# speechcatcher-asr/speechcatcher

Hardware: AMD Instinct MI355X
Metric: concurrent real-time streams (audio-seconds/s), de_xl dims, 640 ms (10240-sample) chunk steps, beam 10 CTC+attention (higher is better)
Workload: dtype f32

## Files before the change

speechcatcher_amd/csrc/gemm.hip:

```cpp
#define SC_STAMP_ON (p.dbg_stamp)
#include "common.h"
#include <mutex>
#include <unordered_map>
#include <vector>

typedef float f32x16 __attribute__((ext_vector_type(16)));
typedef _Float16 h16x4 __attribute__((ext_vector_type(4)));
typedef _Float16 h16x8 __attribute__((ext_vector_type(8)));

__device__ __forceinline__ void ffn_split4(const float4 &x, h16x4 &hi, h16x4 &lo) {
  hi = h16x4{(_Float16)x.x, (_Float16)x.y, (_Float16)x.z, (_Float16)x.w};
  lo = h16x4{(_Float16)((x.x - (float)hi[0]) * 2048.f), (_Float16)((x.y - (float)hi[1]) * 2048.f),
             (_Float16)((x.z - (float)hi[2]) * 2048.f), (_Float16)((x.w - (float)hi[3]) * 2048.f)};
}

struct GemmArgs {
  const float *A;
  const int *a_rows;
  int lda;
  const float *W;
  const float *bias;
  float *C;
  const int *c_rows;
  int ldc;
// ... 745 lines not shown
               "not a tiled problem");
  if (M == 0) return SC_OK;
  hipStream_t st = (hipStream_t)stream;
  resolve_workspace(stream);
  if (sc_hook("SC_GEMM_NAIVE") || sc_hook("SC_SKINNY_MAX_M") || sc_hook("SC_KV_PER_LAYER")) return SC_ERR_ARG;
  ProfScope prof = sc_prof_begin(st);
  GemmArgs g{A, a_rows, lda, W, bias, C, c_rows, ldc, M, N, K, flags, 0, nullptr, K, ncb, cb_stride};
  int ksplit = 0, variant = 0;
  float *ws_keep = g_ws;
  g_ws = nullptr;
  gemm_dispatch(g, false, &ksplit, &variant, st);
  g_ws = ws_keep;
  sc_prof_end(prof, variant, 2.0 * M * N * K, 4.0 * ((double)M * K + (double)N * K + (double)M * N));
  SC_CHECK_LAUNCH();
  return SC_OK;
}

extern "C" int sc_gemm_ln(const float *A, const int32_t *a_rows, int lda, const float *W,
                          const float *bias, float *C, const int32_t *c_rows, int ldc, int M, int N,
                          int K, int flags, int conv_f1, const float *ln_g, const float *ln_b,
                          float ln_eps, float *ln_out, int ld_ln, void *stream) {
  SC_CHECK_ARG(A && W && C && ln_g && ln_b && ln_out, "null pointer");
  SC_CHECK_ARG(M >= 0 && N > 0 && K > 0 && lda > 0 && ldc >= N && ld_ln >= N, "bad dimensions");
  if (M == 0) return SC_OK;
  GemmArgs g{A, a_rows, lda, W, bias, C, c_rows, ldc, M, N, K, flags, conv_f1, nullptr, K};
  hipStream_t st = (hipStream_t)stream;
  resolve_workspace(stream);
  const bool fusable = N <= 1024 && N % 4 == 0 && ld_ln % 4 == 0;
  int ksplit = 0, variant = 0;
  gemm_dispatch(g, fusable, &ksplit, &variant, st);
  if (ksplit > 0 && fusable) {
    gemm_splitk_reduce_ln_kernel<<<cdiv(M, 4), 256, 0, st>>>(g, ksplit, ln_g, ln_b, ln_eps, ln_out, ld_ln);
    SC_CHECK_LAUNCH();
    return SC_OK;
  }
  if (ksplit > 0) {
    const long n4 = (long)M * (N / 4);
    gemm_splitk_reduce_kernel<<<dim3((unsigned)((n4 + 255) / 256)), 256, 0, st>>>(g, ksplit);
  }
  SC_CHECK_LAUNCH();
  return sc_layernorm(C, c_rows, ldc, ln_out, (flags & SC_GEMM_LN_AT_CROWS) ? c_rows : nullptr, ld_ln, M, N, ln_g,
                      ln_b, ln_eps, stream);
}

typedef float f32x4 __attribute__((ext_vector_type(4)));

__device__ __forceinline__ f32x4 ffn_mfma8(f32x4 acc, const float4 &a0, const float4 &a1, const float4 &b0,
                                           const float4 &b1) {
  acc = __builtin_amdgcn_mfma_f32_16x16x4f32(a0.x, b0.x, acc, 0, 0, 0);
  acc = __builtin_amdgcn_mfma_f32_16x16x4f32(a0.y, b0.y, acc, 0, 0, 0);
  acc = __builtin_amdgcn_mfma_f32_16x16x4f32(a0.z, b0.z, acc, 0, 0, 0);
  acc = __builtin_amdgcn_mfma_f32_16x16x4f32(a0.w, b0.w, acc, 0, 0, 0);
  acc = __builtin_amdgcn_mfma_f32_16x16x4f32(a1.x, b1.x, acc, 0, 0, 0);
  acc = __builtin_amdgcn_mfma_f32_16x16x4f32(a1.y, b1.y, acc, 0, 0, 0);
  acc = __builtin_amdgcn_mfma_f32_16x16x4f32(a1.z, b1.z, acc, 0, 0, 0);
  acc = __builtin_amdgcn_mfma_f32_16x16x4f32(a1.w, b1.w, acc, 0, 0, 0);
  return acc;
}

struct FfnArgs {
  const float *XN;
  const int *rows;
  const float *W1p, *b1, *W2p;
  float *part;
  int M, F, cpw;
  const float *PH;
  int nph;
  const float *pbias, *Xin;
  float *Xout;
  const float *g, *b;
  float eps;
  int part_rows;
  int w_form;
  int act_half;
  int dbg_stamp;
  int pgrp;
};

__device__ __forceinline__ f32x4 ffn_mma_h(f32x4 acc, const h16x8 &a, const h16x4 &b0, const h16x4 &b1) {
  acc = __builtin_amdgcn_mfma_f32_16x16x16f16(h16x4{a[0], a[1], a[2], a[3]}, b0, acc, 0, 0, 0);
  acc = __builtin_amdgcn_mfma_f32_16x16x16f16(h16x4{a[4], a[5], a[6], a[7]}, b1, acc, 0, 0, 0);
  return acc;
}
__host__ __device__ static inline size_t ffn_lds_bytes(int D, int RT, bool pro, int wf) {
  const bool wh = wf == 1;
  if (!wh) return (size_t)(RT * (D + 4) + RT * (128 + 4) + (pro ? RT : 0)) * sizeof(float);
  return (size_t)RT * (D + 4) * 4 + (size_t)RT * (D + 8) * 2 + (size_t)RT * (128 + 8) * 2 + (pro ? RT * 4 : 0);
}

template <int D, int RTT, bool PRO = false, int WF = 0>
__global__ __launch_bounds__(512) void ffn_fused_kernel(FfnArgs p) {
  constexpr bool WH = WF == 1, WS = WF == 2;
  constexpr int RT = 16 * RTT, FC = 128;
  constexpr int KI1 = D / 32, KI2 = FC / 32, NT2 = D / 128;
  constexpr int LDX = D + 4, LDH = FC + 4;
  constexpr int LDXH = D + 8, LDHH = FC + 8;
  constexpr int LDXS = 2 * D + 8, LDHS = 2 * FC + 8;
  extern __shared__ __attribute__((aligned(16))) float ffn_smem[];
  float *Xs = ffn_smem;
  float *Hs = ffn_smem + RT * LDX;
  _Float16 *XsH = reinterpret_cast<_Float16 *>(ffn_smem + RT * LDX);
  _Float16 *HsH = XsH + RT * LDXH;
  int *rowid = WH ? reinterpret_cast<int *>(HsH + RT * LDHH)
                  : reinterpret_cast<int *>(ffn_smem + RT * LDX + RT * LDH);
  _Float16 *XsS = reinterpret_cast<_Float16 *>(ffn_smem);
  _Float16 *HsS = reinterpret_cast<_Float16 *>(ffn_smem + RT * LDX);
  typedef typename std::conditional<WS, h16x8, typename std::conditional<WH, h16x4, float4>::type>::type BF;
  auto split_at = [](int c) { return (c >> 3) * 16 + (c & 7); };
  const int lane = threadIdx.x & 63, wave = threadIdx.x >> 6;
  const int r = lane & 15, kk = lane >> 4;
  const int grp = blockIdx.x, m0 = blockIdx.y * RT;
  const int KF = p.F / 32;

  constexpr int NV = RT * D / 4;
  constexpr int NQ = NV / 512;
  static_assert(NV % 512 == 0, "tile must be a multiple of the workgroup");
  SC_STAMP(PRO ? 2 : 3, 0);
  BF bf[KI1][2];
  auto load_b1 = [&](int chunk) {
    const BF *wp = reinterpret_cast<const BF *>(p.W1p) + ((long)(chunk * 8 + wave) * KI1) * 128 + lane;
#pragma unroll
    for (int ki = 0; ki < KI1; ++ki) {
      bf[ki][0] = wp[ki * 128];
      bf[ki][1] = wp[ki * 128 + 64];
    }
  };
  BF b2f[KI2][NT2][2];
  auto load_b2 = [&](int chunk) {
#pragma unroll
    for (int t = 0; t < NT2; ++t) {
      const BF *wp = reinterpret_cast<const BF *>(p.W2p) +
                         ((long)(wave * NT2 + t) * KF + chunk * KI2) * 128 + lane;
#pragma unroll
      for (int k = 0; k < KI2; ++k) {
        b2f[k][t][0] = wp[k * 128];
        b2f[k][t][1] = wp[k * 128 + 64];
      }
    }
  };
  if (PRO) {
    constexpr int C4 = D / 4, Q4 = D / 64;
    const int sub = threadIdx.x & 15;
    float4 gam[Q4], bet[Q4];
#pragma unroll
    for (int q = 0; q < Q4; ++q) {
      gam[q] = *reinterpret_cast<const float4 *>(p.g + 4 * (sub + 16 * q));
      bet[q] = *reinterpret_cast<const float4 *>(p.b + 4 * (sub + 16 * q));
    }
    long rowv[NQ];
#pragma unroll
    for (int q = 0; q < NQ; ++q) {
      const int m = min(m0 + (threadIdx.x + q * 512) / C4, p.M - 1);
      rowv[q] = p.rows ? p.rows[m] : m;
    }
    SC_STAMP_WAIT(2, 1);
#pragma unroll
    for (int q = 0; q < NQ; ++q) {
      const int e = threadIdx.x + q * 512, i = e / C4, c4 = e % C4;
      const long row = rowv[q];
      if (c4 == 0) rowid[i] = (int)row;
      const float4 xi = *reinterpret_cast<const float4 *>(p.Xin + row * D + 4 * c4);
      float4 pb = make_float4(0.f, 0.f, 0.f, 0.f);
      if (p.pbias) pb = *reinterpret_cast<const float4 *>(p.pbias + 4 * c4);
      float4 y = make_float4(0.f, 0.f, 0.f, 0.f);
      auto ldp = [&](long elem) -> float4 {
        if (p.act_half) {
          const h16x4 h = *reinterpret_cast<const h16x4 *>(reinterpret_cast<const _Float16 *>(p.PH) + elem);
          return make_float4((float)h[0], (float)h[1], (float)h[2], (float)h[3]);
        }
        return *reinterpret_cast<const float4 *>(p.PH + elem);
      };
      if (p.pgrp == 1 && p.nph == 2) {
        const float4 p0 = ldp((row * 2) * D + 4 * c4);
        const float4 p1 = ldp((row * 2 + 1) * D + 4 * c4);
        y = sc_add4(p0, p1);
      } else
      for (int z0 = 0; z0 < p.nph; z0 += 8) {
        float4 pv[8];
#pragma unroll
        for (int z = 0; z < 8; ++z) {
          pv[z] = ldp((row * p.nph + min(z0 + z, p.nph - 1)) * D + 4 * c4);
          if (z0 + z >= p.nph) pv[z] = make_float4(0.f, 0.f, 0.f, 0.f);
        }
        if (p.pgrp == 4) {
          const float4 g0 = sc_seq4(pv[0], pv[1], pv[2], pv[3]);
          y = z0 == 0 ? g0 : sc_add4(y, g0);
          if (z0 + 4 < p.nph) y = sc_add4(y, sc_seq4(pv[4], pv[5], pv[6], pv[7]));
        } else {
#pragma unroll
          for (int z = 0; z < 8; ++z)
            if (z0 + z < p.nph) y = (z0 + z == 0) ? pv[0] : sc_add4(y, pv[z]);
        }
      }
      const float4 x = make_float4(xi.x + (y.x + pb.x), xi.y + (y.y + pb.y), xi.z + (y.z + pb.z), xi.w + (y.w + pb.w));
      if (grp == 0 && m0 + i < p.M) *reinterpret_cast<float4 *>(p.Xout + row * D + 4 * c4) = x;
      *reinterpret_cast<float4 *>(Xs + i * LDX + 4 * c4) = x;
    }
    SC_STAMP_WAIT(2, 2);
    load_b1(grp * p.cpw);
    __syncthreads();
    SC_STAMP(2, 3);
    for (int i = threadIdx.x >> 4; i < RT; i += 32) {
      float4 x[Q4];
      float sum = 0.f;
#pragma unroll
      for (int q = 0; q < Q4; ++q) {
        x[q] = *reinterpret_cast<const float4 *>(Xs + i * LDX + 4 * (sub + 16 * q));
        sum += (x[q].x + x[q].y) + (x[q].z + x[q].w);
      }
      const float mean = group_sum<16>(sum) / (float)D;
      float q2 = 0.f;
#pragma unroll
      for (int q = 0; q < Q4; ++q) {
        const float a = x[q].x - mean, b = x[q].y - mean, c = x[q].z - mean, e = x[q].w - mean;
        q2 += (a * a + b * b) + (c * c + e * e);
      }
      const float rstd = 1.0f / sqrtf(group_sum<16>(q2) / (float)D + p.eps);
#pragma unroll
      for (int q = 0; q < Q4; ++q) {
        const float4 o = make_float4((x[q].x - mean) * rstd * gam[q].x + bet[q].x, (x[q].y - mean) * rstd * gam[q].y + bet[q].y,
                                     (x[q].z - mean) * rstd * gam[q].z + bet[q].z, (x[q].w - mean) * rstd * gam[q].w + bet[q].w);
        if (WS) {
          h16x4 hi, lo;
          ffn_split4(o, hi, lo);
          _Float16 *d = XsS + i * LDXS + split_at(4 * (sub + 16 * q));
          *reinterpret_cast<h16x4 *>(d) = hi;
          *reinterpret_cast<h16x4 *>(d + 8) = lo;
        } else if (WH)
          *reinterpret_cast<h16x4 *>(XsH + i * LDXH + 4 * (sub + 16 * q)) =
              h16x4{(_Float16)o.x, (_Float16)o.y, (_Float16)o.z, (_Float16)o.w};
        else
          *reinterpret_cast<float4 *>(Xs + i * LDX + 4 * (sub + 16 * q)) = o;
      }
    }
    SC_STAMP(2, 4);
  } else {
    long rowv[NQ];
#pragma unroll
    for (int q = 0; q < NQ; ++q) {
      const int m = min(m0 + (threadIdx.x + q * 512) / (D / 4), p.M - 1);
      rowv[q] = p.rows ? p.rows[m] : m;
    }
    float4 stage[NQ];
#pragma unroll
    for (int q = 0; q < NQ; ++q)
      stage[q] = *reinterpret_cast<const float4 *>(p.XN + rowv[q] * D + 4 * ((threadIdx.x + q * 512) % (D / 4)));
#pragma unroll
    for (int q = 0; q < NQ; ++q) {
      const int e = threadIdx.x + q * 512;
      if (WS) {
        h16x4 hi, lo;
        ffn_split4(stage[q], hi, lo);
        _Float16 *d = XsS + (e / (D / 4)) * LDXS + split_at(4 * (e % (D / 4)));
        *reinterpret_cast<h16x4 *>(d) = hi;
        *reinterpret_cast<h16x4 *>(d + 8) = lo;
      } else if (WH)
        *reinterpret_cast<h16x4 *>(XsH + (e / (D / 4)) * LDXH + 4 * (e % (D / 4))) =
            h16x4{(_Float16)stage[q].x, (_Float16)stage[q].y, (_Float16)stage[q].z, (_Float16)stage[q].w};
      else
        *reinterpret_cast<float4 *>(Xs + (e / (D / 4)) * LDX + 4 * (e % (D / 4))) = stage[q];
    }
  }
  f32x4 acc2[RTT][NT2];
  f32x4 acc2c[WS ? RTT : 1][WS ? NT2 : 1];
#pragma unroll
  for (int rt = 0; rt < RTT; ++rt)
#pragma unroll
    for (int t = 0; t < NT2; ++t) {
      acc2[rt][t] = f32x4{0.f, 0.f, 0.f, 0.f};
      if (WS) acc2c[rt][t] = f32x4{0.f, 0.f, 0.f, 0.f};
    }

  if (!PRO) load_b1(grp * p.cpw);
  __syncthreads();
  SC_STAMP(PRO ? 2 : 3, PRO ? 5 : 1);
  if (PRO) SC_STAMP_WAIT(2, 6);

  for (int cc = 0; cc < p.cpw; ++cc) {
    const int chunk = grp * p.cpw + cc;
    const float bias = p.b1 ? p.b1[chunk * FC + wave * 16 + r] : 0.f;
    load_b2(chunk);
    f32x4 acc1[RTT];
    f32x4 acc1c[WS ? RTT : 1];
#pragma unroll
    for (int rt = 0; rt < RTT; ++rt) {
      acc1[rt] = f32x4{0.f, 0.f, 0.f, 0.f};
      if (WS) acc1c[rt] = f32x4{0.f, 0.f, 0.f, 0.f};
    }
    if constexpr (WS) {
      constexpr int NS = RTT * KI1;
      const _Float16 *ab = XsS + r * LDXS + 16 * kk;
      h16x8 ah = *reinterpret_cast<const h16x8 *>(ab), al = *reinterpret_cast<const h16x8 *>(ab + 8);
#pragma unroll
      for (int st = 0; st < NS; ++st) {
        const int ki = st / RTT, rt = st % RTT;
        h16x8 nh = ah, nl = al;
        if (st + 1 < NS) {
          const _Float16 *ap = ab + ((st + 1) % RTT) * 16 * LDXS + ((st + 1) / RTT) * 64;
          nh = *reinterpret_cast<const h16x8 *>(ap);
          nl = *reinterpret_cast<const h16x8 *>(ap + 8);
        }
        acc1[rt] = __builtin_amdgcn_mfma_f32_16x16x32_f16(ah, bf[ki][0], acc1[rt], 0, 0, 0);
        acc1c[rt] = __builtin_amdgcn_mfma_f32_16x16x32_f16(ah, bf[ki][1], acc1c[rt], 0, 0, 0);
        acc1c[rt] = __builtin_amdgcn_mfma_f32_16x16x32_f16(al, bf[ki][0], acc1c[rt], 0, 0, 0);
        ah = nh;
        al = nl;
      }
    } else if constexpr (WH) {
      constexpr int NS = RTT * KI1;
      const _Float16 *ab = XsH + r * LDXH + 8 * kk;
      h16x8 a = *reinterpret_cast<const h16x8 *>(ab);
#pragma unroll
      for (int st = 0; st < NS; ++st) {
        const int ki = st / RTT, rt = st % RTT;
        h16x8 n = a;
        if (st + 1 < NS) n = *reinterpret_cast<const h16x8 *>(ab + ((st + 1) % RTT) * 16 * LDXH + ((st + 1) / RTT) * 32);
        acc1[rt] = ffn_mma_h(acc1[rt], a, bf[ki][0], bf[ki][1]);
        a = n;
      }
    } else {
      constexpr int NS = RTT * KI1;
      const float *ab = Xs + r * LDX + 8 * kk;
      float4 a0 = *reinterpret_cast<const float4 *>(ab), a1 = *reinterpret_cast<const float4 *>(ab + 4);
#pragma unroll
      for (int st = 0; st < NS; ++st) {
        const int ki = st / RTT, rt = st % RTT;
        float4 n0 = a0, n1 = a1;
        if (st + 1 < NS) {
          const float *ap = ab + ((st + 1) % RTT) * 16 * LDX + ((st + 1) / RTT) * 32;
          n0 = *reinterpret_cast<const float4 *>(ap);
          n1 = *reinterpret_cast<const float4 *>(ap + 4);
        }
        acc1[rt] = ffn_mfma8(acc1[rt], a0, a1, bf[ki][0], bf[ki][1]);
        a0 = n0;
        a1 = n1;
      }
    }
    if (cc > 0) __syncthreads();
#pragma unroll
    for (int rt = 0; rt < RTT; ++rt)
#pragma unroll
      for (int j = 0; j < 4; ++j) {
        const float hv = fmaxf((WS ? acc1[rt][j] + acc1c[WS ? rt : 0][j] * (1.f / 2048.f) : acc1[rt][j]) + bias, 0.f);
        if (WS) {
          const _Float16 hi = (_Float16)hv;
          _Float16 *d = HsS + (rt * 16 + 4 * kk + j) * LDHS + split_at(wave * 16 + r);
          d[0] = hi;
          d[8] = (_Float16)((hv - (float)hi) * 2048.f);
        } else if (WH) HsH[(rt * 16 + 4 * kk + j) * LDHH + wave * 16 + r] = (_Float16)hv;
        else Hs[(rt * 16 + 4 * kk + j) * LDH + wave * 16 + r] = hv;
      }
    if (cc + 1 < p.cpw) load_b1(chunk + 1);
    __syncthreads();
    const bool tree_last = cc > 0 && cc + 1 == p.cpw;
    if (tree_last) {
#pragma unroll
      for (int rt = 0; rt < RTT; ++rt)
#pragma unroll
        for (int t = 0; t < NT2; ++t) {
#pragma unroll
          for (int j = 0; j < 4; ++j)
            Xs[(rt * 16 + 4 * kk + j) * LDX + (wave * NT2 + t) * 16 + r] =
                WS ? acc2[rt][t][j] + acc2c[WS ? rt : 0][WS ? t : 0][j] * (1.f / 2048.f) : acc2[rt][t][j];
          acc2[rt][t] = f32x4{0.f, 0.f, 0.f, 0.f};
          if (WS) acc2c[WS ? rt : 0][WS ? t : 0] = f32x4{0.f, 0.f, 0.f, 0.f};
        }
    }
    if constexpr (WS) {
      constexpr int NS = RTT * KI2;
      const _Float16 *ab = HsS + r * LDHS + 16 * kk;
      h16x8 ah = *reinterpret_cast<const h16x8 *>(ab), al = *reinterpret_cast<const h16x8 *>(ab + 8);
#pragma unroll
      for (int st = 0; st < NS; ++st) {
        const int k = st / RTT, rt = st % RTT;
        h16x8 nh = ah, nl = al;
        if (st + 1 < NS) {
          const _Float16 *ap = ab + ((st + 1) % RTT) * 16 * LDHS + ((st + 1) / RTT) * 64;
          nh = *reinterpret_cast<const h16x8 *>(ap);
          nl = *reinterpret_cast<const h16x8 *>(ap + 8);
        }
#pragma unroll
        for (int t = 0; t < NT2; ++t) {
          acc2[rt][t] = __builtin_amdgcn_mfma_f32_16x16x32_f16(ah, b2f[k][t][0], acc2[rt][t], 0, 0, 0);
          acc2c[rt][t] = __builtin_amdgcn_mfma_f32_16x16x32_f16(ah, b2f[k][t][1], acc2c[rt][t], 0, 0, 0);
          acc2c[rt][t] = __builtin_amdgcn_mfma_f32_16x16x32_f16(al, b2f[k][t][0], acc2c[rt][t], 0, 0, 0);
        }
        ah = nh;
        al = nl;
      }
    } else if constexpr (WH) {
      constexpr int NS = RTT * KI2;
      const _Float16 *ab = HsH + r * LDHH + 8 * kk;
      h16x8 a = *reinterpret_cast<const h16x8 *>(ab);
#pragma unroll
      for (int st = 0; st < NS; ++st) {
        const int k = st / RTT, rt = st % RTT;
        h16x8 n = a;
        if (st + 1 < NS) n = *reinterpret_cast<const h16x8 *>(ab + ((st + 1) % RTT) * 16 * LDHH + ((st + 1) / RTT) * 32);
#pragma unroll
        for (int t = 0; t < NT2; ++t) acc2[rt][t] = ffn_mma_h(acc2[rt][t], a, b2f[k][t][0], b2f[k][t][1]);
        a = n;
      }
    } else {
      constexpr int NS = RTT * KI2;
      const float *ab = Hs + r * LDH + 8 * kk;
      float4 a0 = *reinterpret_cast<const float4 *>(ab), a1 = *reinterpret_cast<const float4 *>(ab + 4);
#pragma unroll
      for (int st = 0; st < NS; ++st) {
        const int k = st / RTT, rt = st % RTT;
        float4 n0 = a0, n1 = a1;
        if (st + 1 < NS) {
          const float *ap = ab + ((st + 1) % RTT) * 16 * LDH + ((st + 1) / RTT) * 32;
          n0 = *reinterpret_cast<const float4 *>(ap);
          n1 = *reinterpret_cast<const float4 *>(ap + 4);
        }
#pragma unroll
        for (int t = 0; t < NT2; ++t) acc2[rt][t] = ffn_mfma8(acc2[rt][t], a0, a1, b2f[k][t][0], b2f[k][t][1]);
        a0 = n0;
        a1 = n1;
      }
    }
  }
#pragma unroll
  for (int rt = 0; rt < RTT; ++rt)
#pragma unroll
    for (int t = 0; t < NT2; ++t)
#pragma unroll
      for (int j = 0; j < 4; ++j) {
        float *xp = Xs + (rt * 16 + 4 * kk + j) * LDX + (wave * NT2 + t) * 16 + r;
        const float v = WS ? acc2[rt][t][j] + acc2c[WS ? rt : 0][WS ? t : 0][j] * (1.f / 2048.f) : acc2[rt][t][j];
        *xp = p.cpw > 1 ? *xp + v : v;
      }
  __syncthreads();
  SC_STAMP(PRO ? 2 : 3, PRO ? 7 : 2);
  float *dst = p.part + ((long)grp * p.M + m0) * D;
#pragma unroll
  for (int q = 0; q < NQ; ++q) {
    const int e = threadIdx.x + q * 512;
    const int i = e / (D / 4), c4 = e % (D / 4);
    if (m0 + i < p.M) {
      const float4 v = *reinterpret_cast<const float4 *>(Xs + i * LDX + 4 * c4);
      if (PRO && p.act_half) {
        *reinterpret_cast<h16x4 *>(reinterpret_cast<_Float16 *>(p.part) + ((long)grp * p.part_rows + rowid[i]) * D + 4 * c4) =
            h16x4{(_Float16)v.x, (_Float16)v.y, (_Float16)v.z, (_Float16)v.w};
      } else {
        float *o = PRO ? p.part + ((long)grp * p.part_rows + rowid[i]) * D : dst + (long)i * D;
        if (!PRO && p.part_rows > 0) o = p.part + ((long)grp * p.part_rows + (p.rows ? p.rows[m0 + i] : m0 + i)) * D;
        *reinterpret_cast<float4 *>(o + 4 * c4) = v;
      }
    }
  }
  SC_STAMP_END(PRO ? 2 : 3, PRO ? 8 : 3);
}
SC_PHASE_GETTER(sc_phase_debug_ffn)

template <int D, int RTT, bool PRO, int WH>
static void launch_ffn_wh(const FfnArgs &p, int ngrp, hipStream_t st) {
  constexpr int RT = 16 * RTT;
  const size_t lds = ffn_lds_bytes(D, RT, PRO, WH);
  static bool attr_done = false;
  if (!attr_done && lds > 64 * 1024) {
    (void)hipFuncSetAttribute(reinterpret_cast<const void *>(&ffn_fused_kernel<D, RTT, PRO, WH>),
                              hipFuncAttributeMaxDynamicSharedMemorySize, (int)lds);
    attr_done = true;
  }
  ffn_fused_kernel<D, RTT, PRO, WH><<<dim3(ngrp, cdiv(p.M, RT)), 512, lds, st>>>(p);
}
template <int D, int RTT, bool PRO = false>
static void launch_ffn(const FfnArgs &p, int ngrp, hipStream_t st) {
  if (p.w_form == 2) launch_ffn_wh<D, RTT, PRO, 2>(p, ngrp, st);
  else if (p.w_form) launch_ffn_wh<D, RTT, PRO, 1>(p, ngrp, st);
  else launch_ffn_wh<D, RTT, PRO, 0>(p, ngrp, st);
}

template <int D, bool PRO = false>
static void launch_ffn_rtt(const FfnArgs &p, int rtt, int ngrp, hipStream_t st) {
  switch (rtt) {
    case 1: launch_ffn<D, 1, PRO>(p, ngrp, st); break;
    case 2: launch_ffn<D, 2, PRO>(p, ngrp, st); break;
    case 3: launch_ffn<D, 3, PRO>(p, ngrp, st); break;
    case 4: launch_ffn<D, 4, PRO>(p, ngrp, st); break;
    default: launch_ffn<D, 5, PRO>(p, ngrp, st); break;
  }
}

struct RowProjArgs {
  const float *A;
  int lda;
  const float *ln_g, *ln_b;
  const float *Wp, *bias;
  const float *R;
  float *C;
  int ldc;
  const float *g2, *b2;
  float *LN2;
  float eps;
  int M, N, cpw;
  int w_form;
};

template <int D>
__device__ __forceinline__ float4 rowtile_ln(const float4 v, bool act, const float *g, const float *b, float eps,
                                             int lane) {
  float s = act ? (v.x + v.y) + (v.z + v.w) : 0.f;
  const float mean = wave_sum(s) / (float)D;
  const float a = v.x - mean, bb = v.y - mean, c = v.z - mean, e = v.w - mean;
  const float q = act ? (a * a + bb * bb) + (c * c + e * e) : 0.f;
  const float rstd = 1.0f / sqrtf(wave_sum(q) / (float)D + eps);
  float4 o = v;
  if (act) {
    const float4 gm = reinterpret_cast<const float4 *>(g)[lane];
    const float4 bt = reinterpret_cast<const float4 *>(b)[lane];
    o = make_float4(a * rstd * gm.x + bt.x, bb * rstd * gm.y + bt.y, c * rstd * gm.z + bt.z, e * rstd * gm.w + bt.w);
  }
  return o;
}

template <int D, int RTT, bool FULL, int WF = 0>
__global__ __launch_bounds__(512) void rowtile_proj_kernel(RowProjArgs p) {
  constexpr bool WH = WF == 1, WS = WF == 2;
  constexpr int RT = 16 * RTT, FC = 128, KI1 = D / 32;
  constexpr int LDXS = 2 * D + 8;
  constexpr int LDX = D + 4, LDO = FULL ? D + 4 : FC + 4;
  constexpr int LDXH = D + 8;
  extern __shared__ __attribute__((aligned(16))) float rowtile_smem[];
  float *Xs = rowtile_smem;
  float *Os = rowtile_smem + RT * LDX;
  _Float16 *XsH = reinterpret_cast<_Float16 *>(rowtile_smem + RT * LDX + RT * LDO);
  _Float16 *XsS = reinterpret_cast<_Float16 *>(rowtile_smem);
  typedef typename std::conditional<WS, h16x8, typename std::conditional<WH, h16x4, float4>::type>::type BF;
  const int lane = threadIdx.x & 63, wave = threadIdx.x >> 6;
  const int r = lane & 15, kk = lane >> 4;
  const int grp = blockIdx.x, m0 = blockIdx.y * RT;
  const int nch = FULL ? D / FC : p.cpw, ch0 = FULL ? 0 : grp * p.cpw;

  BF bf[KI1][2];
  auto load_b = [&](int chunk) {
    const BF *wp = reinterpret_cast<const BF *>(p.Wp) + ((long)(chunk * 8 + wave) * KI1) * 128 + lane;
#pragma unroll
    for (int ki = 0; ki < KI1; ++ki) {
      bf[ki][0] = wp[ki * 128];
      bf[ki][1] = wp[ki * 128 + 64];
    }
  };
  load_b(ch0);
  constexpr int NV = RT * D / 4, NQ = NV / 512;
  static_assert(NV % 512 == 0, "tile must be a multiple of the workgroup");
  {
    float4 stage[NQ];
#pragma unroll
    for (int q = 0; q < NQ; ++q) {
      const int e = threadIdx.x + q * 512;
      const int m = min(m0 + e / (D / 4), p.M - 1);
      stage[q] = *reinterpret_cast<const float4 *>(p.A + (long)m * p.lda + 4 * (e % (D / 4)));
// ... 153 lines not shown

template <int D, bool FULL>
static void launch_rowtile_rtt(const RowProjArgs &p, int rtt, int ngrp, hipStream_t st) {
  switch (rtt) {
    case 1: launch_rowtile<D, 1, FULL>(p, ngrp, st); break;
    case 2: launch_rowtile<D, 2, FULL>(p, ngrp, st); break;
    case 3: launch_rowtile<D, 3, FULL>(p, ngrp, st); break;
    default: launch_rowtile<D, 4, FULL>(p, ngrp, st); break;
  }
}

extern "C" int sc_rowtile_proj_supported(int D, int N) {
  return (D == 256 || D == 128) && N % 128 == 0 && N >= 128;
}

static int rowtile_run(const float *A, int lda, int M, int D, const float *ln_g, const float *ln_b,
                       float eps, const float *Wp, const float *bias, int N, const float *R, float *C,
                       int ldc, const float *g2, const float *b2, float *LN2, void *stream, int w_form) {
  SC_CHECK_ARG(A && Wp && C, "null pointer");
  SC_CHECK_ARG(sc_rowtile_proj_supported(D, N), "unsupported dimensions");
  SC_CHECK_ARG((!ln_g) == (!ln_b) && (!LN2 || (g2 && b2)), "LayerNorm parameters missing");
  const bool full = R || LN2;
  SC_CHECK_ARG(!full || N == D, "residual / output LayerNorm need N == D");
  SC_CHECK_ARG(lda % 4 == 0 && ldc % 4 == 0 && lda >= D && ldc >= N, "leading dimensions");
  SC_CHECK_ARG((((uintptr_t)A | (uintptr_t)Wp | (uintptr_t)C | (uintptr_t)R | (uintptr_t)LN2) & 15) == 0,
               "16-byte alignment");
  if (M <= 0) return SC_OK;
  hipStream_t st = (hipStream_t)stream;
  const int nch = N / 128;
  int best_rtt = 1, best_cpw = full ? nch : 1;
  double best = 1e30;
  for (int cpw = full ? nch : 1; cpw <= nch; ++cpw) {
    if (nch % cpw) continue;
    for (int rtt = 1; rtt <= 4; ++rtt) {
      const long wgs = (long)(nch / cpw) * cdiv(M, 16 * rtt);
      const int conc = (rtt <= 3 && wgs > 256) ? 2 : 1;
      const double t_wg = (4.3 + 1.0 * rtt + 2.1 * rtt * cpw) * (rtt == 4 ? 1.08 : 1.0);
      const double t = (double)((wgs + 256 * conc - 1) / (256 * conc)) * t_wg * (conc == 2 ? 1.75 : 1.0);
      if (t < best) { best = t; best_rtt = rtt; best_cpw = cpw; }
    }
  }
  if (const char *f = sc_hook("SC_ROWTILE_FORCE")) {
    int r = 0, c = 0;
    if (sscanf(f, "%d,%d", &r, &c) == 2 && r >= 1 && r <= 4 && c >= 1 && nch % c == 0) {
      best_rtt = r;
      if (!full) best_cpw = c;
    }
  }
  RowProjArgs p{A, lda, ln_g, ln_b, Wp, bias, R, C, ldc, g2, b2, LN2, eps, M, N, best_cpw, w_form};
  ProfScope prof = sc_prof_begin(st);
  const int ngrp = full ? 1 : nch / best_cpw;
  if (D == 256) {
    if (full) launch_rowtile_rtt<256, true>(p, best_rtt, ngrp, st);
    else launch_rowtile_rtt<256, false>(p, best_rtt, ngrp, st);
  } else {
    if (full) launch_rowtile_rtt<128, true>(p, best_rtt, ngrp, st);
    else launch_rowtile_rtt<128, false>(p, best_rtt, ngrp, st);
  }
  sc_prof_end(prof, SC_PROF_ROWTILE_PROJ, 2.0 * (double)M * D * N,
              4.0 * ((double)M * (D + N) + (double)D * N / (w_form == 1 ? 2.0 : 1.0) + (full ? 2.0 * M * D : 0.0)));
  SC_CHECK_LAUNCH();
  return SC_OK;
}

extern "C" int sc_rowtile_proj(const float *A, int lda, int M, int D, const float *ln_g, const float *ln_b,
                               float eps, const float *Wp, const float *bias, int N, const float *R, float *C,
                               int ldc, const float *g2, const float *b2, float *LN2, void *stream) {
  return rowtile_run(A, lda, M, D, ln_g, ln_b, eps, Wp, bias, N, R, C, ldc, g2, b2, LN2, stream, 0);
}
extern "C" int sc_rowtile_proj_h(const float *A, int lda, int M, int D, const float *ln_g, const float *ln_b,
                                 float eps, const void *Wh, const float *bias, int N, const float *R, float *C,
                                 int ldc, const float *g2, const float *b2, float *LN2, void *stream) {
  return rowtile_run(A, lda, M, D, ln_g, ln_b, eps, reinterpret_cast<const float *>(Wh), bias, N, R, C, ldc, g2, b2, LN2,
                     stream, 1);
}

extern "C" int sc_rowtile_proj_s(const float *A, int lda, int M, int D, const float *ln_g, const float *ln_b,
                                 float eps, const void *Ws, const float *bias, int N, const float *R, float *C,
                                 int ldc, const float *g2, const float *b2, float *LN2, void *stream) {
  return rowtile_run(A, lda, M, D, ln_g, ln_b, eps, reinterpret_cast<const float *>(Ws), bias, N, R, C, ldc, g2, b2, LN2,
                     stream, 2);
}


static inline int ffn_rtt_max(int D, int w_form) { return (w_form == 2 && D == 256) ? 3 : 5; }

extern "C" int sc_ffn_ln_supported(int D, int F) { return (D == 256 || D == 128) && F % 128 == 0 && F >= 128; }

static int ffn_run(const float *XN, const int32_t *rows, int M, int D, int F, const float *W1p,
                   const float *b1, const float *W2p, const float *b2, float *X, const float *ln_g,
                   const float *ln_b, float ln_eps, float *ln_out, float *Xout, const float *Wq,
                   const float *bq, float *Q, int N, void *stream, int w_form = 0,
                   const ScHandoff *ho = nullptr) {
  SC_CHECK_ARG(XN && W1p && W2p && X, "null pointer");
  SC_CHECK_ARG(sc_ffn_ln_supported(D, F), "unsupported dimensions");
  SC_CHECK_ARG(!ln_out || (ln_g && ln_b), "LayerNorm parameters missing");
  SC_CHECK_ARG((((uintptr_t)XN | (uintptr_t)W1p | (uintptr_t)W2p | (uintptr_t)X) & 15) == 0, "16-byte alignment");
  if (M <= 0) return SC_OK;
  hipStream_t st = (hipStream_t)stream;
  resolve_workspace(stream);
  SC_CHECK_ARG(g_ws && g_ws_bytes >= (size_t)16 * D * sizeof(float), "sc_ffn_ln needs the split-K workspace");
  const int nch = F / 128;
  const long ws_rows_per_part = (long)(g_ws_bytes / sizeof(float) / D);
  int m_done = 0;
  while (m_done < M) {
    int best_rtt = 5, best_cpw = nch;
    long slab = M - m_done;
    double best = 1e30;
    for (int cpw = 1; cpw <= 2; cpw *= 2) {
      if (nch % cpw) continue;
      const int ngrp = nch / cpw;
      long fit = ws_rows_per_part / ngrp;
      if (fit < 16) continue;
      const long mm = fit < (M - m_done) ? (fit / 80) * 80 : (M - m_done);
      if (mm <= 0) continue;
      for (int rtt = 1; rtt <= ffn_rtt_max(D, w_form); ++rtt) {
        const long wgs = (long)ngrp * ((mm + 16 * rtt - 1) / (16 * rtt));
        const double rounds = (double)((wgs + 255) / 256);
        double t = rounds * (2.5 + 4.0 * rtt * cpw) + 1.5 + 2.0 * (double)mm * D * 4.0 * ngrp / 3.0e6;
        t *= (double)(M - m_done) / (double)mm;
        if (t < best) { best = t; best_rtt = rtt; best_cpw = cpw; slab = mm; }
      }
    }
    SC_CHECK_ARG(best < 1e29, "workspace too small for sc_ffn_ln");
    SC_CHECK_ARG(!Wq || slab == M, "workspace too small for the fused projection (rows do not fit one slab)");
    SC_CHECK_ARG(!ho || (slab == M && !rows && !ln_out && !Wq), "context hand-off: all rows in one slab, no row table / LayerNorm");
    if (const char *f = sc_hook("SC_FFN_FORCE")) {
      int r = 0, c = 0;
      if (sscanf(f, "%d,%d", &r, &c) == 2 && r >= 1 && r <= 5 && c >= 1 && c <= 2 && nch % c == 0 &&
          (long)(M - m_done) * (nch / c) <= ws_rows_per_part) {
        best_rtt = r;
        best_cpw = c;
        slab = M - m_done;
      }
    }
    const int ngrp = nch / best_cpw;
    FfnArgs p{XN, rows ? rows + m_done : nullptr, W1p, b1, W2p, g_ws, (int)slab, F, best_cpw};
    p.w_form = w_form;
    p.dbg_stamp = sc_phase_take(3);
    const float *xn_base = rows ? XN : XN + (long)m_done * D;
    p.XN = xn_base;
    ProfScope prof = sc_prof_begin(st);
    if (D == 256) launch_ffn_rtt<256>(p, best_rtt, ngrp, st);
    else launch_ffn_rtt<128>(p, best_rtt, ngrp, st);
    sc_prof_end(prof, SC_PROF_FFN_FUSED, 4.0 * (double)slab * D * F,
                4.0 * (2.0 * (double)slab * D + 2.0 * (double)D * F));
    SC_CHECK_LAUNCH();
    GemmArgs g{nullptr, nullptr, D, nullptr, b2, rows ? X : X + (long)m_done * D, rows ? rows + m_done : nullptr, D,
               (int)slab, D, F, SC_GEMM_RESIDUAL | (rows ? SC_GEMM_LN_AT_CROWS : 0), 0, g_ws, 0};
    if (Wq) {
      int rc = sc_launch_reduce_ln_proj(g_ws, ngrp, (int)slab, b2, X, Xout, rows, M, D, ln_g, ln_b, ln_eps, ln_out,
                                        Wq, bq, Q, N, st);
      if (rc != SC_OK) return rc;
    } else if (ho) {
      const long n4 = (long)slab * (D / 4);
      ffn_reduce_handoff_kernel<<<dim3((unsigned)((n4 + 255) / 256)), 256, 0, st>>>(g, ngrp, *ho);
    } else if (ln_out) {
      float *lo = rows ? ln_out : ln_out + (long)m_done * D;
      gemm_splitk_reduce_ln_kernel<<<cdiv((int)slab, 4), 256, 0, st>>>(g, ngrp, ln_g, ln_b, ln_eps, lo, D);
    } else {
      const long n4 = (long)slab * (D / 4);
      gemm_splitk_reduce_kernel<<<dim3((unsigned)((n4 + 255) / 256)), 256, 0, st>>>(g, ngrp);
    }
    SC_CHECK_LAUNCH();
    m_done += (int)slab;
  }
  return SC_OK;
}

extern "C" int sc_ffn_ln(const float *XN, const int32_t *rows, int M, int D, int F, const float *W1p,
                         const float *b1, const float *W2p, const float *b2, float *X, const float *ln_g,
                         const float *ln_b, float ln_eps, float *ln_out, void *stream) {
  return ffn_run(XN, rows, M, D, F, W1p, b1, W2p, b2, X, ln_g, ln_b, ln_eps, ln_out, nullptr, nullptr, nullptr,
                 nullptr, 0, stream);
}

int sc_ffn_ln_handoff(const float *XN, int M, int D, int F, const void *W1, const float *b1, const void *W2, const float *b2,
                      float *X, int w_form, const ScHandoff &ho, void *stream) {
  SC_CHECK_ARG(ho.blkinfo && ho.state && ho.R > 1 && M % ho.R == 0, "hand-off table");
  return ffn_run(XN, nullptr, M, D, F, (const float *)W1, b1, (const float *)W2, b2, X, nullptr, nullptr, 0.f, nullptr, nullptr,
                 nullptr, nullptr, nullptr, 0, stream, w_form, &ho);
}

extern "C" int sc_ffn_ln_h(const float *XN, const int32_t *rows, int M, int D, int F, const void *W1h,
                           const float *b1, const void *W2h, const float *b2, float *X, const float *ln_g,
                           const float *ln_b, float ln_eps, float *ln_out, void *stream) {
  return ffn_run(XN, rows, M, D, F, (const float *)W1h, b1, (const float *)W2h, b2, X, ln_g, ln_b, ln_eps, ln_out, nullptr,
                 nullptr, nullptr, nullptr, 0, stream, 1);
}
extern "C" int sc_ffn_ln_s(const float *XN, const int32_t *rows, int M, int D, int F, const void *W1s,
                           const float *b1, const void *W2s, const float *b2, float *X, const float *ln_g,
                           const float *ln_b, float ln_eps, float *ln_out, void *stream) {
  return ffn_run(XN, rows, M, D, F, (const float *)W1s, b1, (const float *)W2s, b2, X, ln_g, ln_b, ln_eps, ln_out, nullptr,
                 nullptr, nullptr, nullptr, 0, stream, 2);
}
extern "C" int sc_ffn_ln_proj_s(const float *XN, const int32_t *rows, int M, int D, int F, const void *W1s,
                                const float *b1, const void *W2s, const float *b2, const float *Xin, float *Xout,
                                const float *ln_g, const float *ln_b, float ln_eps, float *ln_out, const float *Wq,
                                const float *bq, float *Q, int N, void *stream) {
  SC_CHECK_ARG(Xin && Xout && Xin != Xout && Wq && Q && ln_g && ln_b, "null / aliased operand");
  SC_CHECK_ARG(sc_proj_ln_proj_supported(D) && N > 0 && N % D == 0, "projection width must be a multiple of D");
  return ffn_run(XN, rows, M, D, F, (const float *)W1s, b1, (const float *)W2s, b2, const_cast<float *>(Xin), ln_g, ln_b,
                 ln_eps, ln_out, Xout, Wq, bq, Q, N, stream, 2);
}
extern "C" int sc_ffn_ln_proj_h(const float *XN, const int32_t *rows, int M, int D, int F, const void *W1h,
                                const float *b1, const void *W2h, const float *b2, const float *Xin, float *Xout,
                                const float *ln_g, const float *ln_b, float ln_eps, float *ln_out, const float *Wq,
                                const float *bq, float *Q, int N, void *stream) {
  SC_CHECK_ARG(Xin && Xout && Xin != Xout && Wq && Q && ln_g && ln_b, "null / aliased operand");
  SC_CHECK_ARG(sc_proj_ln_proj_supported(D) && N > 0 && N % D == 0, "projection width must be a multiple of D");
  return ffn_run(XN, rows, M, D, F, (const float *)W1h, b1, (const float *)W2h, b2, const_cast<float *>(Xin), ln_g, ln_b,
                 ln_eps, ln_out, Xout, Wq, bq, Q, N, stream, 1);
// ... 118 lines not shown
```

Before: 4075.

## Double-buffer FFN hidden tile and keep first-chunk partials in registers

The fused FFN kernel now gives each of the two hidden chunks its own LDS slot when they fit within a 160 KB budget. This removes the extra barrier between chunks, and the first chunk's second-GEMM partial sums stay in registers instead of being written back into the X tile. Row ids are now always recorded in LDS so the output store has a single addressing path. The split-precision form with D=256 is capped at RTT 2 to make room for the larger footprint. In exchange the kernel uses more LDS and registers, which may lower occupancy and narrows the autotune search.

Measured after the change: 4105, median of 6. No clear change (+0.7%).

```diff
diff --git a/speechcatcher_amd/csrc/gemm.hip b/speechcatcher_amd/csrc/gemm.hip
--- a/speechcatcher_amd/csrc/gemm.hip
+++ b/speechcatcher_amd/csrc/gemm.hip
@@ -851,11 +851,12 @@
   acc = __builtin_amdgcn_mfma_f32_16x16x16f16(h16x4{a[4], a[5], a[6], a[7]}, b1, acc, 0, 0, 0);
   return acc;
 }
-__host__ __device__ static inline size_t ffn_lds_bytes(int D, int RT, bool pro, int wf) {
-  const bool wh = wf == 1;
-  if (!wh) return (size_t)(RT * (D + 4) + RT * (128 + 4) + (pro ? RT : 0)) * sizeof(float);
-  return (size_t)RT * (D + 4) * 4 + (size_t)RT * (D + 8) * 2 + (size_t)RT * (128 + 8) * 2 + (pro ? RT * 4 : 0);
-}
+static constexpr size_t FFN_LDS_MAX = 160 * 1024;
+__host__ __device__ static constexpr size_t ffn_lds_bytes(int D, int RT, int wf, int nslot = 1) {
+  return wf == 1 ? (size_t)RT * (D + 4) * 4 + RT * 4 + (size_t)RT * (D + 8) * 2 + (size_t)nslot * RT * (128 + 8) * 2
+                 : (size_t)(RT * (D + 4) + RT + nslot * RT * (128 + 4)) * sizeof(float);
+}
+__host__ __device__ static constexpr bool ffn_two_slots(int D, int RT, int wf) { return ffn_lds_bytes(D, RT, wf, 2) <= FFN_LDS_MAX; }
 
 template <int D, int RTT, bool PRO = false, int WF = 0>
 __global__ __launch_bounds__(512) void ffn_fused_kernel(FfnArgs p) {
@@ -865,15 +866,15 @@
   constexpr int LDX = D + 4, LDH = FC + 4;
   constexpr int LDXH = D + 8, LDHH = FC + 8;
   constexpr int LDXS = 2 * D + 8, LDHS = 2 * FC + 8;
+  const bool two_slots = ffn_two_slots(D, RT, WF) && p.cpw > 1;
   extern __shared__ __attribute__((aligned(16))) float ffn_smem[];
   float *Xs = ffn_smem;
-  float *Hs = ffn_smem + RT * LDX;
-  _Float16 *XsH = reinterpret_cast<_Float16 *>(ffn_smem + RT * LDX);
+  int *rowid = reinterpret_cast<int *>(ffn_smem + RT * LDX);
+  float *Hs = ffn_smem + RT * LDX + RT;
+  _Float16 *XsH = reinterpret_cast<_Float16 *>(ffn_smem + RT * LDX + RT);
   _Float16 *HsH = XsH + RT * LDXH;
-  int *rowid = WH ? reinterpret_cast<int *>(HsH + RT * LDHH)
-                  : reinterpret_cast<int *>(ffn_smem + RT * LDX + RT * LDH);
   _Float16 *XsS = reinterpret_cast<_Float16 *>(ffn_smem);
-  _Float16 *HsS = reinterpret_cast<_Float16 *>(ffn_smem + RT * LDX);
+  _Float16 *HsS = reinterpret_cast<_Float16 *>(Hs);
   typedef typename std::conditional<WS, h16x8, typename std::conditional<WH, h16x4, float4>::type>::type BF;
   auto split_at = [](int c) { return (c >> 3) * 16 + (c & 7); };
   const int lane = threadIdx.x & 63, wave = threadIdx.x >> 6;
@@ -1017,6 +1018,7 @@
 #pragma unroll
     for (int q = 0; q < NQ; ++q) {
       const int e = threadIdx.x + q * 512;
+      if (e % (D / 4) == 0) rowid[e / (D / 4)] = (int)rowv[q];
       if (WS) {
         h16x4 hi, lo;
         ffn_split4(stage[q], hi, lo);
@@ -1032,6 +1034,8 @@
   }
   f32x4 acc2[RTT][NT2];
   f32x4 acc2c[WS ? RTT : 1][WS ? NT2 : 1];
+  constexpr bool KEEP = ffn_two_slots(D, RT, WF);
+  f32x4 keep[KEEP ? RTT : 1][KEEP ? NT2 : 1];
 #pragma unroll
   for (int rt = 0; rt < RTT; ++rt)
 #pragma unroll
@@ -1049,6 +1053,9 @@
     const int chunk = grp * p.cpw + cc;
     const float bias = p.b1 ? p.b1[chunk * FC + wave * 16 + r] : 0.f;
     load_b2(chunk);
+    const int slot = two_slots ? cc : 0;
+    float *Hc = Hs + slot * RT * LDH;
+    _Float16 *HcH = HsH + slot * RT * LDHH, *HcS = HsS + slot * RT * LDHS;
     f32x4 acc1[RTT];
     f32x4 acc1c[WS ? RTT : 1];
 #pragma unroll
@@ -1105,7 +1112,22 @@
         a1 = n1;
       }
     }
-    if (cc > 0) __syncthreads();
+    if (cc > 0 && !two_slots) {
+      __syncthreads();
+      if constexpr (!KEEP) {
+#pragma unroll
+        for (int rt = 0; rt < RTT; ++rt)
+#pragma unroll
+          for (int t = 0; t < NT2; ++t) {
+#pragma unroll
+            for (int j = 0; j < 4; ++j)
+              Xs[(rt * 16 + 4 * kk + j) * LDX + (wave * NT2 + t) * 16 + r] =
+                  WS ? acc2[rt][t][j] + acc2c[WS ? rt : 0][WS ? t : 0][j] * (1.f / 2048.f) : acc2[rt][t][j];
+            acc2[rt][t] = f32x4{0.f, 0.f, 0.f, 0.f};
+            if (WS) acc2c[WS ? rt : 0][WS ? t : 0] = f32x4{0.f, 0.f, 0.f, 0.f};
+          }
+      }
+    }
 #pragma unroll
     for (int rt = 0; rt < RTT; ++rt)
 #pragma unroll
@@ -1113,31 +1135,17 @@
         const float hv = fmaxf((WS ? acc1[rt][j] + acc1c[WS ? rt : 0][j] * (1.f / 2048.f) : acc1[rt][j]) + bias, 0.f);
         if (WS) {
           const _Float16 hi = (_Float16)hv;
-          _Float16 *d = HsS + (rt * 16 + 4 * kk + j) * LDHS + split_at(wave * 16 + r);
+          _Float16 *d = HcS + (rt * 16 + 4 * kk + j) * LDHS + split_at(wave * 16 + r);
           d[0] = hi;
           d[8] = (_Float16)((hv - (float)hi) * 2048.f);
-        } else if (WH) HsH[(rt * 16 + 4 * kk + j) * LDHH + wave * 16 + r] = (_Float16)hv;
-        else Hs[(rt * 16 + 4 * kk + j) * LDH + wave * 16 + r] = hv;
+        } else if (WH) HcH[(rt * 16 + 4 * kk + j) * LDHH + wave * 16 + r] = (_Float16)hv;
+        else Hc[(rt * 16 + 4 * kk + j) * LDH + wave * 16 + r] = hv;
       }
     if (cc + 1 < p.cpw) load_b1(chunk + 1);
     __syncthreads();
-    const bool tree_last = cc > 0 && cc + 1 == p.cpw;
-    if (tree_last) {
-#pragma unroll
-      for (int rt = 0; rt < RTT; ++rt)
-#pragma unroll
-        for (int t = 0; t < NT2; ++t) {
-#pragma unroll
-          for (int j = 0; j < 4; ++j)
-            Xs[(rt * 16 + 4 * kk + j) * LDX + (wave * NT2 + t) * 16 + r] =
-                WS ? acc2[rt][t][j] + acc2c[WS ? rt : 0][WS ? t : 0][j] * (1.f / 2048.f) : acc2[rt][t][j];
-          acc2[rt][t] = f32x4{0.f, 0.f, 0.f, 0.f};
-          if (WS) acc2c[WS ? rt : 0][WS ? t : 0] = f32x4{0.f, 0.f, 0.f, 0.f};
-        }
-    }
     if constexpr (WS) {
       constexpr int NS = RTT * KI2;
-      const _Float16 *ab = HsS + r * LDHS + 16 * kk;
+      const _Float16 *ab = HcS + r * LDHS + 16 * kk;
       h16x8 ah = *reinterpret_cast<const h16x8 *>(ab), al = *reinterpret_cast<const h16x8 *>(ab + 8);
 #pragma unroll
       for (int st = 0; st < NS; ++st) {
@@ -1159,7 +1167,7 @@
       }
     } else if constexpr (WH) {
       constexpr int NS = RTT * KI2;
-      const _Float16 *ab = HsH + r * LDHH + 8 * kk;
+      const _Float16 *ab = HcH + r * LDHH + 8 * kk;
       h16x8 a = *reinterpret_cast<const h16x8 *>(ab);
 #pragma unroll
       for (int st = 0; st < NS; ++st) {
@@ -1172,7 +1180,7 @@
       }
     } else {
       constexpr int NS = RTT * KI2;
-      const float *ab = Hs + r * LDH + 8 * kk;
+      const float *ab = Hc + r * LDH + 8 * kk;
       float4 a0 = *reinterpret_cast<const float4 *>(ab), a1 = *reinterpret_cast<const float4 *>(ab + 4);
 #pragma unroll
       for (int st = 0; st < NS; ++st) {
@@ -1189,6 +1197,18 @@
         a1 = n1;
       }
     }
+    if (KEEP && cc == 0 && p.cpw > 1) {
+#pragma unroll
+      for (int rt = 0; rt < RTT; ++rt)
+#pragma unroll
+        for (int t = 0; t < NT2; ++t) {
+#pragma unroll
+          for (int j = 0; j < 4; ++j)
+            keep[KEEP ? rt : 0][KEEP ? t : 0][j] = WS ? acc2[rt][t][j] + acc2c[WS ? rt : 0][WS ? t : 0][j] * (1.f / 2048.f) : acc2[rt][t][j];
+          acc2[rt][t] = f32x4{0.f, 0.f, 0.f, 0.f};
+          if (WS) acc2c[WS ? rt : 0][WS ? t : 0] = f32x4{0.f, 0.f, 0.f, 0.f};
+        }
+    }
   }
 #pragma unroll
   for (int rt = 0; rt < RTT; ++rt)
@@ -1196,27 +1216,24 @@
     for (int t = 0; t < NT2; ++t)
 #pragma unroll
       for (int j = 0; j < 4; ++j) {
+        const float c = WS ? acc2[rt][t][j] + acc2c[WS ? rt : 0][WS ? t : 0][j] * (1.f / 2048.f) : acc2[rt][t][j];
         float *xp = Xs + (rt * 16 + 4 * kk + j) * LDX + (wave * NT2 + t) * 16 + r;
-        const float v = WS ? acc2[rt][t][j] + acc2c[WS ? rt : 0][WS ? t : 0][j] * (1.f / 2048.f) : acc2[rt][t][j];
-        *xp = p.cpw > 1 ? *xp + v : v;
+        *xp = p.cpw > 1 ? (KEEP ? keep[KEEP ? rt : 0][KEEP ? t : 0][j] : *xp) + c : c;
       }
   __syncthreads();
   SC_STAMP(PRO ? 2 : 3, PRO ? 7 : 2);
-  float *dst = p.part + ((long)grp * p.M + m0) * D;
 #pragma unroll
   for (int q = 0; q < NQ; ++q) {
     const int e = threadIdx.x + q * 512;
     const int i = e / (D / 4), c4 = e % (D / 4);
     if (m0 + i < p.M) {
       const float4 v = *reinterpret_cast<const float4 *>(Xs + i * LDX + 4 * c4);
-      if (PRO && p.act_half) {
-        *reinterpret_cast<h16x4 *>(reinterpret_cast<_Float16 *>(p.part) + ((long)grp * p.part_rows + rowid[i]) * D + 4 * c4) =
+      const long orow = (PRO || p.part_rows > 0) ? (long)grp * p.part_rows + rowid[i] : (long)grp * p.M + m0 + i;
+      if (PRO && p.act_half)
+        *reinterpret_cast<h16x4 *>(reinterpret_cast<_Float16 *>(p.part) + orow * D + 4 * c4) =
             h16x4{(_Float16)v.x, (_Float16)v.y, (_Float16)v.z, (_Float16)v.w};
-      } else {
-        float *o = PRO ? p.part + ((long)grp * p.part_rows + rowid[i]) * D : dst + (long)i * D;
-        if (!PRO && p.part_rows > 0) o = p.part + ((long)grp * p.part_rows + (p.rows ? p.rows[m0 + i] : m0 + i)) * D;
-        *reinterpret_cast<float4 *>(o + 4 * c4) = v;
-      }
+      else
+        *reinterpret_cast<float4 *>(p.part + orow * D + 4 * c4) = v;
     }
   }
   SC_STAMP_END(PRO ? 2 : 3, PRO ? 8 : 3);
@@ -1226,19 +1243,22 @@
 template <int D, int RTT, bool PRO, int WH>
 static void launch_ffn_wh(const FfnArgs &p, int ngrp, hipStream_t st) {
   constexpr int RT = 16 * RTT;
-  const size_t lds = ffn_lds_bytes(D, RT, PRO, WH);
+  const size_t lds = ffn_lds_bytes(D, RT, WH, ffn_two_slots(D, RT, WH) && p.cpw > 1 ? 2 : 1);
+  constexpr size_t lds_max = ffn_lds_bytes(D, RT, WH, ffn_two_slots(D, RT, WH) ? 2 : 1);
   static bool attr_done = false;
-  if (!attr_done && lds > 64 * 1024) {
+  if (!attr_done && lds_max > 64 * 1024) {
     (void)hipFuncSetAttribute(reinterpret_cast<const void *>(&ffn_fused_kernel<D, RTT, PRO, WH>),
-                              hipFuncAttributeMaxDynamicSharedMemorySize, (int)lds);
+                              hipFuncAttributeMaxDynamicSharedMemorySize, (int)lds_max);
     attr_done = true;
   }
   ffn_fused_kernel<D, RTT, PRO, WH><<<dim3(ngrp, cdiv(p.M, RT)), 512, lds, st>>>(p);
 }
+__host__ __device__ static constexpr int ffn_rtt_max(int D, int w_form) { return (w_form == 2 && D == 256) ? 2 : 5; }
 template <int D, int RTT, bool PRO = false>
 static void launch_ffn(const FfnArgs &p, int ngrp, hipStream_t st) {
-  if (p.w_form == 2) launch_ffn_wh<D, RTT, PRO, 2>(p, ngrp, st);
-  else if (p.w_form) launch_ffn_wh<D, RTT, PRO, 1>(p, ngrp, st);
+  if (p.w_form == 2) {
+    if constexpr (RTT <= ffn_rtt_max(D, 2)) launch_ffn_wh<D, RTT, PRO, 2>(p, ngrp, st);
+  } else if (p.w_form) launch_ffn_wh<D, RTT, PRO, 1>(p, ngrp, st);
   else launch_ffn_wh<D, RTT, PRO, 0>(p, ngrp, st);
 }
 
@@ -1558,8 +1578,6 @@
                      stream, 2);
 }
 
-
-static inline int ffn_rtt_max(int D, int w_form) { return (w_form == 2 && D == 256) ? 3 : 5; }
 
 extern "C" int sc_ffn_ln_supported(int D, int F) { return (D == 256 || D == 128) && F % 128 == 0 && F >= 128; }
 
@@ -1603,7 +1621,7 @@
     SC_CHECK_ARG(!ho || (slab == M && !rows && !ln_out && !Wq), "context hand-off: all rows in one slab, no row table / LayerNorm");
     if (const char *f = sc_hook("SC_FFN_FORCE")) {
       int r = 0, c = 0;
-      if (sscanf(f, "%d,%d", &r, &c) == 2 && r >= 1 && r <= 5 && c >= 1 && c <= 2 && nch % c == 0 &&
+      if (sscanf(f, "%d,%d", &r, &c) == 2 && r >= 1 && r <= ffn_rtt_max(D, w_form) && c >= 1 && c <= 2 && nch % c == 0 &&
           (long)(M - m_done) * (nch / c) <= ws_rows_per_part) {
         best_rtt = r;
         best_cpw = c;
```
